# Neptune-Crypto/twenty-first

Hardware: AMD Instinct MI355X
Metric: goldilocks_ntt_gfelts_per_s (higher is better)
Workload: dtype u64

## Files before the change

include/tf_hip.h:

```cpp
#ifndef TF_HIP_H
#define TF_HIP_H

#include <stddef.h>
#include <stdint.h>

#ifdef __cplusplus
extern "C" {
#endif

enum tf_status {
    TF_OK = 0,
    TF_ERR_TOO_FEW_LEAFS = 1,
    TF_ERR_INCORRECT_NUMBER_OF_LEAFS = 2,
    TF_ERR_TREE_TOO_HIGH = 3,
    TF_ERR_LEN_NOT_POWER_OF_TWO = 4,
    TF_ERR_LEN_TOO_LARGE = 5,
    TF_ERR_ORDER_NOT_ABOVE_DEGREE = 6,
    TF_ERR_NULL_POINTER = 7,
    TF_ERR_NO_DEVICE = 8,
    TF_ERR_HIP = 9,
    TF_ERR_OUT_OF_MEMORY = 10,
    TF_ERR_LEAF_INDEX_INVALID = 11,
    TF_ERR_INVERSE_OF_ZERO = 12,
    TF_ERR_BUFFER_TOO_SMALL = 13,
// ... 198 lines not shown
int tf_tip5_sponge_sample_indices(uint64_t *states, size_t count, uint32_t upper_bound, size_t num_indices, uint32_t *out_u32);
int tf_tip5_sponge_sample_indices_dev(uint64_t *d_states, size_t count, uint32_t upper_bound, size_t num_indices, uint32_t *d_out_u32,
                                      void *stream);

int tf_batch_inversion_bfe(const uint64_t *in, size_t n, uint64_t *out);
int tf_batch_inversion_xfe(const uint64_t *in, size_t n, uint64_t *out);
int tf_batch_inversion_bfe_dev(const uint64_t *d_in, size_t n, uint64_t *d_out, void *stream);
int tf_batch_inversion_xfe_dev(const uint64_t *d_in, size_t n, uint64_t *d_out, void *stream);
int tf_batch_inversion_bfe_dev_async(const uint64_t *d_in, size_t n, uint64_t *d_out, void *stream, int *d_status);
int tf_batch_inversion_xfe_dev_async(const uint64_t *d_in, size_t n, uint64_t *d_out, void *stream, int *d_status);
int tf_inverse_or_zero_bfe(const uint64_t *in, size_t n, uint64_t *out);
int tf_inverse_or_zero_xfe(const uint64_t *in, size_t n, uint64_t *out);
int tf_inverse_or_zero_bfe_dev(const uint64_t *d_in, size_t n, uint64_t *d_out, void *stream);
int tf_inverse_or_zero_xfe_dev(const uint64_t *d_in, size_t n, uint64_t *d_out, void *stream);

void tf_set_ntt_tile_bytes(size_t bytes);
size_t tf_get_ntt_tile_bytes(void);
void tf_set_ntt_pipe(int streams);
int tf_get_ntt_pipe(void);

void tf_set_ntt_min_passes(int passes);
void tf_set_ntt_small_launch(int mode);
void tf_set_ntt_two_pass(int mode);
void tf_set_ntt_latency_kernel(int mode);
int tf_ntt_launch_count(size_t n, size_t batch, int width);
int tf_ntt_plan(size_t n, int width, int* log2_radix_out);
double tf_debug_sclk_mhz(void);

#ifdef TF_AB_BUILD
void tf_set_ntt_nt(int mask);
void tf_set_ntt_chain(int tiles_per_workgroup);
int tf_debug_stamps(unsigned long long *host_out, size_t words);
#endif
int tf_debug_fill_random_dev(uint64_t *d_out, size_t count, uint64_t seed, uint64_t first_index, void *stream);

#ifdef __cplusplus
}
#endif
#endif
```

twenty-first_amd/_lib.py:

```python
from __future__ import annotations

import ctypes as C
import os
import subprocess

_HERE = os.path.dirname(os.path.abspath(__file__))
SO_PATH = os.environ.get("TF_HIP_LIBRARY") or os.path.join(_HERE, "libtf_hip.so")
HEADER = os.path.join(os.path.dirname(_HERE), "include", "tf_hip.h")

_u64p = C.POINTER(C.c_uint64)
_sz = C.c_size_t
_vp = C.c_void_p

SIGNATURES = {
    "tf_status_string": (C.c_char_p, [C.c_int]),
    "tf_last_error": (C.c_char_p, []),
    "tf_version": (C.c_int, []),
    "tf_source_hash": (C.c_char_p, []),
    "tf_device_count": (C.c_int, []),
    "tf_set_device": (C.c_int, [C.c_int]),
    "tf_get_device": (C.c_int, [C.POINTER(C.c_int)]),
    "tf_shard_range": (C.c_int, [_sz, C.c_int, C.c_int, C.POINTER(_sz), C.POINTER(_sz)]),
    "tf_merkle_multi_subtrees": (C.c_int, [_sz, _sz, C.c_int]),
    "tf_prepare_ntt": (C.c_int, [_sz, _sz, C.c_int, C.c_int]),
# ... 131 lines not shown
    "tf_tip5_sponge_squeeze": (C.c_int, [_vp, _sz, _sz, _vp]),
    "tf_tip5_sponge_squeeze_dev": (C.c_int, [_vp, _sz, _sz, _vp, _vp]),
    "tf_tip5_sponge_sample_scalars": (C.c_int, [_vp, _sz, _sz, _vp]),
    "tf_tip5_sponge_sample_scalars_dev": (C.c_int, [_vp, _sz, _sz, _vp, _vp]),
    "tf_tip5_sponge_sample_indices": (C.c_int, [_vp, _sz, C.c_uint32, _sz, _vp]),
    "tf_tip5_sponge_sample_indices_dev": (C.c_int, [_vp, _sz, C.c_uint32, _sz, _vp, _vp]),
    "tf_merkle_verify_proofs": (C.c_int, [_vp, _sz, _vp, _vp, _vp, _vp, _vp, _vp, _vp]),
    "tf_merkle_verify_proofs_dev": (C.c_int, [_vp, _sz, _vp, _vp, _vp, _vp, _vp, _vp, _vp, _vp]),
    "tf_merkle_authentication_paths": (C.c_int, [_vp, _sz, _vp, _vp, _vp, _vp, _vp, _vp, _vp]),
    "tf_merkle_authentication_paths_dev": (C.c_int, [_vp, _sz, _vp, _vp, _vp, _vp, _vp, _vp, _vp, _vp]),
    "tf_ntt_launch_count": (C.c_int, [_sz, _sz, C.c_int]),
    "tf_ntt_plan": (C.c_int, [_sz, C.c_int, C.POINTER(C.c_int)]),
    "tf_batch_eval_plan": (C.c_int, [_sz, _sz, _sz, C.c_int]),
    "tf_poly_interpolate_bfe_dev_async": (C.c_int, [_vp, _vp, _sz, _sz, _vp, _vp, _vp]),
    "tf_poly_interpolate_xfe_dev_async": (C.c_int, [_vp, _vp, _sz, _sz, _vp, _vp, _vp]),
    "tf_poly_clean_divide_bfe_dev_async": (C.c_int, [_vp, _sz, _vp, _sz, _vp, _vp, _vp]),
    "tf_poly_clean_divide_many_bfe_dev_async": (C.c_int, [_vp, _sz, _sz, _vp, _sz, _vp, _vp, _vp]),
    "tf_zerofier_tree_new_bfe_dev_async": (C.c_int, [_vp, _sz, _vp, C.POINTER(C.c_void_p)]),
    "tf_zerofier_tree_new_xfe_dev_async": (C.c_int, [_vp, _sz, _vp, C.POINTER(C.c_void_p)]),
    "tf_zerofier_tree_interpolate_dev_async": (C.c_int, [_vp, _vp, _sz, _vp, _vp, _vp]),
    "tf_release_caches": (C.c_int, []),
    "tf_set_ntt_small_launch": (None, [C.c_int]),
    "tf_set_ntt_two_pass": (None, [C.c_int]),
    "tf_set_ntt_latency_kernel": (None, [C.c_int]),
    "tf_debug_sclk_mhz": (C.c_double, []),
    "tf_set_ntt_tile_bytes": (None, [_sz]),
    "tf_set_ntt_min_passes": (None, [C.c_int]),
    "tf_get_ntt_tile_bytes": (_sz, []),
    "tf_set_ntt_pipe": (None, [C.c_int]),
    "tf_get_ntt_pipe": (C.c_int, []),
    "tf_set_batch_eval_route": (None, [C.c_int]),
    "tf_debug_fill_random_dev": (C.c_int, [_vp, _sz, C.c_uint64, C.c_uint64, _vp]),
}


AB_SIGNATURES = {
    "tf_set_ntt_chain": (None, [C.c_int]),
    "tf_debug_stamps": (C.c_int, [_vp, _sz]),
    "tf_set_ntt_nt": (None, [C.c_int]),
}


def build(force: bool = False) -> str:
    csrc = os.path.join(_HERE, "csrc")
    args = ["make", "-C", csrc]
    if force:
# ... 57 lines not shown
```

twenty-first_amd/csrc/ntt_kernels.h:

```cpp
#pragma once

#include <type_traits>

#include "gl64.h"
#include "ntt_args.h"
#include "ntt_network.h"

namespace tfk {

using gl::u32;
using gl::u64;

struct NttPassArgs {
    const u64* in;
    u64* out;
    const u64* inner_tw;
    const u64* post_tw;
    const u64* pre_scale;
    long long n_out;
    const u64* in2;
    const u64* post_scale;
    long long js_i0, js_i1, js_i2, js_c, js_k;
    long long n_coeffs;
    long long ps_i1;
// ... 147 lines not shown
                           Pre2Slot<INV, Q0 + 3>::neg ? v3[3] : v2[3]};
        const u64 m0[4] = {Pre2Slot<INV, Q0>::neg ? v0[0] : v1[0], Pre2Slot<INV, Q0 + 1>::neg ? v0[1] : v1[1], Pre2Slot<INV, Q0 + 2>::neg ? v0[2] : v1[2],
                           Pre2Slot<INV, Q0 + 3>::neg ? v0[3] : v1[3]};
        const u64 m1[4] = {Pre2Slot<INV, Q0>::neg ? v2[0] : v3[0], Pre2Slot<INV, Q0 + 1>::neg ? v2[1] : v3[1], Pre2Slot<INV, Q0 + 2>::neg ? v2[2] : v3[2],
                           Pre2Slot<INV, Q0 + 3>::neg ? v2[3] : v3[3]};
        gl::add_lazy4(p0, p1, t);
        gl::sub_lazy4(t, m0, u);
        gl::sub_lazy4(u, m1, t);
        pre4_shift4<INV, Q0>(x, t);
    } else {
        constexpr int E4 = TwExp<INV, 2, 1>::value;
        gl::sub_lazy4(v0, v2, t);
        gl::sub_lazy4(v1, v3, u);
        const u64 w[4] = {gl::Pow2Mul<E4>::apply(u[0]), gl::Pow2Mul<E4>::apply(u[1]), gl::Pow2Mul<E4>::apply(u[2]), gl::Pow2Mul<E4>::apply(u[3])};
        if ((cls == 1) != gl::Pow2Mul<E4>::negate) gl::add_lazy4(t, w, u);
        else gl::sub_lazy4(t, w, u);
        const u64 b4[4] = {stw[brev5(Q0)], stw[brev5(Q0 + 1)], stw[brev5(Q0 + 2)], stw[brev5(Q0 + 3)]};
        gl::mont_mul4(u, b4, t);
        x[Q0] = t[0], x[Q0 + 1] = t[1], x[Q0 + 2] = t[2], x[Q0 + 3] = t[3];
    }
}
#endif

template <bool INV, int SCALE, int MODE = 0, bool LAST1024 = false, bool R1024 = false, bool COL = false, bool PRE2 = false, bool PRE4 = false>
#ifndef TF_PRIO_LOAD
#define TF_PRIO_LOAD 3
#endif
#ifndef TF_PRIO_STEP2
#define TF_PRIO_STEP2 0
#endif
#ifndef TF_NTT_WAVES
#define TF_NTT_WAVES 4
#endif
__global__ void __launch_bounds__(512, TF_NTT_WAVES) ntt_pass_kernel(const NttPassArgs A) {
    extern __shared__ __attribute__((aligned(16))) u64 lds[];
    const int t = threadIdx.x;
    const int p2 = (LAST1024 || R1024) ? 5 : A.p2;
    const int P2 = 1 << p2;
    constexpr bool COLP = R1024 || COL;
    constexpr bool LAZY1 = (LAST1024 || COLP) && MODE != 2;
    constexpr bool LAZY2 = COLP && MODE == 0;
    const int L = A.L;

    static_assert(!PRE2 || ((LAST1024 || R1024) && MODE == 0 && SCALE != 3), "PRE2 is a variant of the R = 1024 kernels");
    static_assert(!PRE4 || (LAST1024 && !PRE2 && !INV && MODE == 0 && SCALE == 0), "PRE4 is a variant of the plain forward R = 1024 last pass");
#ifndef TF_AB_BUILD
    static_assert(!PRE4, "the radix-4 last pass is a measured loss: laboratory build only");
#endif
    u32 bid = blockIdx.x, half = 0;
    if constexpr (PRE2) {
        if (A.pre2_map == 1) half = (bid >> 3) & 1u, bid = (bid & 7u) | ((bid >> 4) << 3);
        else half = bid & 1u, bid >>= 1;
    }
    if constexpr (PRE4) {
        if (A.pre2_map == 1) half = (bid >> 3) & 3u, bid = (bid & 7u) | ((bid >> 5) << 3);
        else half = bid & 3u, bid >>= 2;
    }
    u32 i0, i1, i2;
    if (A.xcd_order) {
        const u32 G = (u32)A.xcd_order;
        const u32 xcd = bid & 7u, slot = bid >> 3;
        const u32 ngrp = A.d2 / (8u * G);
        const u32 grp = A.xcd_colfast ? slot % ngrp : slot / (G * A.d01);
        const u32 within = A.xcd_colfast ? slot / ngrp : slot % (G * A.d01);
#ifndef TF_XCD_SKEW
#define TF_XCD_SKEW 0
#endif
#ifndef TF_NAT_SKEW
#define TF_NAT_SKEW 0
#endif
        i2 = ((grp << 3) | (TF_XCD_SKEW ? ((xcd + grp * TF_XCD_SKEW) & 7u) : xcd)) * G + within % G;
        const u32 rest = within / G;
        i1 = rest % A.d1;
        i0 = rest / A.d1;
    } else {
        const u32 tile = bid;
        i2 = tile % A.d2;
        const u32 rest = tile / A.d2;
        i1 = rest % A.d1;
        i0 = rest / A.d1;
        if (TF_NAT_SKEW && (A.d2 & 7u) == 0) i2 = (i2 & ~7u) | ((i2 + (i2 >> 3) * TF_NAT_SKEW + rest * TF_NAT_SKEW) & 7u);
    }
    const u64* in = A.in + (long long)i0 * A.ib0 + (long long)i1 * A.ib1 + (long long)i2 * A.ib2;
    u64* out = A.out + (long long)i0 * A.ob0 + (long long)i1 * A.ob1 + (long long)i2 * A.ob2;
    const bool wt = LAST1024 || A.wtiles;
    const int cshift = LAST1024 ? (int)((A.col_shift0 + i0 * (u32)A.col_shift_i0) & 15u) : 0;
    constexpr bool GEO = R1024;
    const int nc_ = GEO ? kR1024Nc : A.nc;
    const int cpr_ = GEO ? kR1024Cpr : A.cpr, nrounds_ = GEO ? kR1024Rounds : A.nrounds;
    const int s1_ = GEO ? kR1024S1 : A.s1, s2_ = GEO ? kR1024Cpr : A.s2, s3_ = GEO ? 1 : A.s3;
    const int col0 = (int)i2 * nc_ - cshift;
    const int ncv = min(nc_, A.col_limit - col0);
    const int ch0 = wt ? (int)div_by_L((u32)max(col0, 0), L) : 0;
    if (wt) {
        in = A.in + (long long)i0 * A.ib0 + (long long)i1 * A.ib1 + (long long)ch0 * A.in_cs_hi;
        out = A.out + (long long)i0 * A.ob0 + (long long)i1 * A.ob1 + (long long)ch0 * A.out_cs_hi;
    }
    if constexpr (PRE2 || PRE4) out += (long long)half * A.pre2_out_off;

    const int g = (LAST1024 || GEO) ? (t >> 4) : (A.gfast ? (t & (P2 - 1)) : (A.nc == 1 ? t : (int)__umulhi((u32)t, A.nc_magic)));
    const int c = (LAST1024 || GEO) ? (t & 15) : (A.gfast ? (t >> p2) : (t - g * A.nc));
    const bool act = c < ncv;
    int ch, cl;
    if (wt) {
        const int w = col0 + c + ((LAST1024 && col0 + c < 0) ? A.col_wrap : 0);
        const int e = (int)div_by_L((u32)w, L);
        ch = e - ch0, cl = w - e * L;
    } else {
        ch = (int)div_by_L((u32)c, L), cl = c - ch * L;
    }
    const long long bcol = (long long)div_by_L((u32)max(col0 + c, 0), L);
    int g_in = LAST1024 ? ((t & 7) | ((t >> 1) & 0x18)) : g;
    int c_in = LAST1024 ? (((t >> 6) & 7) | (t & 8)) : c;
#ifndef TF_XFE_ROLES
#define TF_XFE_ROLES 1
#endif
    if constexpr (LAST1024 && TF_XFE_ROLES) {
        if (L == 3 && col0 >= 0) {
            const int r = (t >> 3) & 1;
            const int v = (t & 7) | ((t >> 4) << 3);
            const int wc0 = col0 + 8 * r;
            int nk = 3 - (wc0 - 3 * (int)div_by_L((u32)wc0, 3));
            int start = 0, colbase = 0;
#pragma unroll
            for (int k = 0; k < 3; ++k) {
                if (v >= start + 32 * nk) {
                    start += 32 * nk;
                    colbase += nk;
                    nk = min(3, 8 - colbase);
                }
            }
            const int local = v - start;
            const int gq = nk == 1 ? local : (nk == 2 ? (local >> 1) : (int)__umulhi((u32)local, 0x55555556u));
            g_in = gq;
            c_in = 8 * r + colbase + (local - gq * nk);
        }
    }
    const bool act_in = LAST1024 ? (c_in < ncv) : act;
    int ch_in = ch, cl_in = cl;
    if constexpr (LAST1024) {
        const int w = col0 + c_in + (col0 + c_in < 0 ? A.col_wrap : 0);
        const int e = (int)div_by_L((u32)w, L);
        ch_in = e - ch0, cl_in = w - e * L;
    }

    unsigned long long stamp[6];
    if constexpr (MODE == 3) stamp[0] = __builtin_readcyclecounter();
    u64 x[32];
#pragma unroll
    for (int q = 0; q < 32; ++q) x[q] = 0;
    constexpr bool LDS_TW = TF_LDS_TW && MODE == 0;
    u64* const ltw = lds + (LAST1024 ? kL1024ExchangeWords : 32 * s1_);
    if constexpr (LDS_TW) {
        if ((LAST1024 || R1024) || A.inner_tw) {
            const u64* itw = A.inner_tw + ((PRE2 || PRE4) ? (int)half * 1024 : 0);
            for (int i = t; i < 32 * P2; i += blockDim.x) ltw[(i >> 5) * kLdsTwStride + (i & 31)] = itw[i];
            __syncthreads();
        }
    }
    __builtin_amdgcn_s_setprio(TF_PRIO_LOAD);
    if constexpr (MODE == 1) {
#pragma unroll
        for (int q = 0; q < 32; ++q) x[q] = (u64)(t * 32 + q) * 0x9e3779b97f4a7c15ULL >> 1;
#ifdef TF_AB_BUILD
    } else if (PRE4 && act_in) {
        const u32 toff = (u32)(((long long)ch_in * A.in_cs_hi + cl_in + (long long)g_in * A.in_rs) * 8);
        const __amdgpu_buffer_rsrc_t ri = buf_rsrc(in);
        const u32 poff = (u32)(A.pre2_in_off * 8);
        const auto slot_off = [&](int q) { return (u32)((long long)(brev5(q) << p2) * A.in_rs * 8); };
        const auto ld = [&](u32 so) { return buf_load<0>(ri, toff, so); };
        const u64* stw = A.pre4_stw + (half >> 1) * 32;
        const auto group = [&](auto q0c) {
            constexpr int Q0 = decltype(q0c)::value;
            u64 v0[4], v1[4], v2[4], v3[4];
#pragma unroll
            for (int i = 0; i < 4; ++i) {
                const u32 so = slot_off(Q0 + i);
                v0[i] = ld(so), v1[i] = ld(so + poff), v2[i] = ld(so + 2 * poff), v3[i] = ld(so + 3 * poff);
            }
            pre4_combine4<INV, Q0>(x, v0, v1, v2, v3, half, stw);
        };
        group(std::integral_constant<int, 0>{});
        group(std::integral_constant<int, 4>{});
// ... 112 lines not shown
        }
        } else {
#pragma unroll
        for (int q = 0; q < 32; ++q) x[q] = ld(slot_off(q));
#pragma unroll
        for (int q0 = 0; q0 < 32; q0 += 8) {
            u64 w[8];
#pragma unroll
            for (int i = 0; i < 8; ++i) w[i] = ld(slot_off(q0 + i) + poff);
            scale8(w);
            if (q0 == 0) pre2_combine8<INV, 0>(x, w, half != 0);
            else if (q0 == 8) pre2_combine8<INV, 8>(x, w, half != 0);
            else if (q0 == 16) pre2_combine8<INV, 16>(x, w, half != 0);
            else pre2_combine8<INV, 24>(x, w, half != 0);
        }
        }
    } else if (act_in) {
        const u32 toff = (u32)(((long long)ch_in * A.in_cs_hi + cl_in + (long long)g_in * A.in_rs) * 8);
        const char* base = reinterpret_cast<const char*>(in);
        if constexpr ((LAST1024 || COLP) && SCALE != 1) {
            const __amdgpu_buffer_rsrc_t ri = buf_rsrc(in);
#pragma unroll
            for (int q = 0; q < 32; ++q) x[q] = buf_load<LAST1024 ? TF_AUX_LAST_LOAD : TF_LOAD_AUX>(ri, toff, (u32)((long long)(brev5(q) << p2) * A.in_rs * 8));
        } else
#pragma unroll
        for (int q = 0; q < 32; ++q) {
            const long long ur = (long long)(brev5(q) << p2);
            const u64* ptr = reinterpret_cast<const u64*>(base + ur * A.in_rs * 8 + toff);
            if constexpr (SCALE == 1) {
                const long long j = (ur + g) * A.ps_rs + (A.ps_col ? bcol : 0);
                if (A.n_coeffs < 0 || j < A.n_coeffs) x[q] = *ptr;
            } else {
#ifdef TF_AB_BUILD
                x[q] = (A.nt & 1) ? __builtin_nontemporal_load(ptr) : *ptr;
#else
                x[q] = *ptr;
#endif
            }
        }
    }
    if constexpr (SCALE == 1) {
        if (act_in && A.in2) {
            const char* base2 = reinterpret_cast<const char*>(in + (A.in2 - A.in));
            const u32 toff2 = (u32)(((long long)ch_in * A.in_cs_hi + cl_in + (long long)g_in * A.in_rs) * 8);
#pragma unroll
            for (int q0 = 0; q0 < 32; q0 += 8) {
// ... 18 lines not shown
                    const long long j = (ur + g) * A.ps_rs + (A.ps_col ? bcol : 0);
                    w[i] = ps[j < A.n_coeffs ? j : 0];
                }
#pragma unroll
                for (int i = 0; i < 8; i += 4) mul4_inplace(x, q0 + i, w[i], w[i + 1], w[i + 2], w[i + 3]);
            }
        }
    }
    if constexpr (PRE2 && !(TF_PRE2_BURST16 == 2 && SCALE != 1)) {
        if (half && act_in) pre2_shift<INV>(x);
    }
    __builtin_amdgcn_s_setprio(0);
    if constexpr (MODE != 2 && !(PRE2 && TF_PRE2_BURST16 == 2 && SCALE != 1)) {
        dit_half<INV, 0, LAZY1>(x);
        __builtin_amdgcn_sched_barrier(0);
    }
    if constexpr (MODE == 3) {
        stamp[1] = __builtin_readcyclecounter();
        asm volatile("s_waitcnt vmcnt(0)" ::: "memory");
        stamp[2] = __builtin_readcyclecounter();
    }
    if constexpr (MODE != 2) {
        dit_half<INV, 16, LAZY1>(x);
        dit_level<INV, 5, LAZY1>(x);
        if ((LAST1024 || R1024) || A.inner_tw) {
            const u64* tw = LDS_TW ? ltw + g_in * kLdsTwStride : A.inner_tw + g_in * 32;
#pragma unroll
            for (int q = 0; q < 32; q += 4) mul4_inplace(x, q, tw[q], tw[q + 1], tw[q + 2], tw[q + 3]);
        }
    }
    if constexpr (MODE == 3) { asm volatile("" :: "v"(x[0]), "v"(x[31])); stamp[3] = __builtin_readcyclecounter(); }
    if constexpr (LAST1024) {
        constexpr int S1 = kL1024S1, CS = kL1024CS;
        const int wround = c_in >> 3, wcc = c_in & 7, rround = c >> 3, rcc = c & 7;
        u64* wr = lds + wcc * CS + g_in;
        const u64* rd = lds + g * S1 + rcc * CS;
        const int nr = (A.nc + 7) >> 3;
#pragma unroll 1
        for (int r = 0; r < nr; ++r) {
            if (r) __syncthreads();
            if (wround == r) {
#pragma unroll
                for (int q = 0; q < 32; ++q) wr[q * S1] = x[q];
            }
            __syncthreads();
            if (rround == r) {
#pragma unroll
                for (int q = 0; q < 32; ++q) x[q] = rd[brev5(q)];
            }
        }
    } else if (p2 != 0) {
        const int myround = c / cpr_;
        const int cc = c - myround * cpr_;
        u64* wr = lds + g * s2_ + cc * s3_;
        const u64* rd = lds + cc * s3_;
#pragma unroll 1
        for (int r = 0; r < nrounds_; ++r) {
            if (r) __syncthreads();
            if (myround == r) {
#pragma unroll
// ... 10 lines not shown
                    x[q] = rd[k1 * s1_ + gg * s2_];
                }
            }
        }
    }
    if constexpr (MODE == 3) { asm volatile("" :: "v"(x[0]), "v"(x[31])); stamp[4] = __builtin_readcyclecounter(); }
    __builtin_amdgcn_s_setprio(TF_PRIO_STEP2);
    if constexpr (LAST1024) {
        dit_half<INV, 0>(x);
        dit_half<INV, 16>(x);
        const u32 toff = (u32)(((long long)ch * A.out_cs_hi + cl + (long long)g * A.out_rs) * 8);
        char* base = reinterpret_cast<char*>(out);
        if constexpr (SCALE == 2) {
            long long j0 = (long long)i0 * A.js_i0 + (long long)i1 * A.js_i1 + (long long)(ch0 + ch) * A.js_c + (long long)g * A.js_k;
            if constexpr (PRE2) j0 += (long long)half * A.pre2_js_off;
            const char* sb = reinterpret_cast<const char*>(A.post_scale);
            const u32 soff = (u32)(j0 * 8);
            tail_p5<INV, 0, false, true>(x, act, base, toff, A.out_rs * 8, 32, sb, soff, A.js_k * 8);
            tail_p5<INV, 4, false, true>(x, act, base, toff, A.out_rs * 8, 32, sb, soff, A.js_k * 8);
            tail_p5<INV, 8, false, true>(x, act, base, toff, A.out_rs * 8, 32, sb, soff, A.js_k * 8);
            tail_p5<INV, 12, false, true>(x, act, base, toff, A.out_rs * 8, 32, sb, soff, A.js_k * 8);
            return;
        }
        if (A.n_out >= 0) {
            const long long j0 = (long long)i0 * A.js_i0 + (long long)i1 * A.js_i1 + (long long)(ch0 + ch) * A.js_c + (long long)g * A.js_k;
            const long long rem = A.n_out - j0, step = 32 * A.js_k;
            const int qlim = rem <= 0 ? 0 : (int)min(32ll, (rem + step - 1) / step);
            tail_p5<INV, 0, true>(x, act, base, toff, A.out_rs * 8, qlim);
            tail_p5<INV, 4, true>(x, act, base, toff, A.out_rs * 8, qlim);
            tail_p5<INV, 8, true>(x, act, base, toff, A.out_rs * 8, qlim);
            tail_p5<INV, 12, true>(x, act, base, toff, A.out_rs * 8, qlim);
            return;
        }
        const bool nts = (A.nt & 2) != 0;
        tail_p5<INV, 0>(x, act, base, toff, A.out_rs * 8, 32, nullptr, 0, 0, nts);
        tail_p5<INV, 4>(x, act, base, toff, A.out_rs * 8, 32, nullptr, 0, 0, nts);
        tail_p5<INV, 8>(x, act, base, toff, A.out_rs * 8, 32, nullptr, 0, 0, nts);
        tail_p5<INV, 12>(x, act, base, toff, A.out_rs * 8, 32, nullptr, 0, 0, nts);
        return;
    }
    if constexpr (MODE != 2) {
        if (p2 >= 1) dit_level<INV, 1, LAZY2>(x);
        if (p2 >= 2) dit_level<INV, 2, LAZY2>(x);
        if (p2 >= 3) dit_level<INV, 3, LAZY2>(x);
        if (p2 >= 4) dit_level<INV, 4, LAZY2>(x);
        if (p2 >= 5) dit_level<INV, 5, LAZY2>(x);
    }
// ... 944 lines not shown
```

twenty-first_amd/csrc/tf_abi.hip:

```cpp
#include "tf_internal.h"
#include "aux_kernels.h"

#include <functional>

namespace tfi {

struct DevBuf {
    u64* p = nullptr;
    hipStream_t s;
    explicit DevBuf(hipStream_t st) : s(st) {}
    int alloc(size_t words) {
        if (words == 0) return TF_OK;
        hipError_t e = pool_malloc_async(reinterpret_cast<void**>(&p), words * sizeof(u64), s);
        if (e != hipSuccess) return hip_fail(e, "hipMallocAsync", __FILE__, __LINE__);
        return TF_OK;
    }
    ~DevBuf() {
        if (p) (void)hipFreeAsync(p, s);
    }
};

int h2d(u64* d, const u64* h, size_t words, hipStream_t s) {
    if (!words) return TF_OK;
    HIPCHK(hipMemcpyAsync(d, h, words * sizeof(u64), hipMemcpyHostToDevice, s));
// ... 227 lines not shown
    return TF_OK;
} TF_ABI_CATCH

#ifdef TF_AB_BUILD
int tf_debug_stamps(unsigned long long* host_out, size_t words) try {
    if (!g_dbg_buf) {
        if (hipMalloc(reinterpret_cast<void**>(&g_dbg_buf), 4096 * 8 * 6 * 8) != hipSuccess) return TF_ERR_HIP;
        (void)hipMemset(g_dbg_buf, 0, 4096 * 8 * 6 * 8);
    }
    if (host_out && words) {
        if (hipDeviceSynchronize() != hipSuccess) return TF_ERR_HIP;
        if (hipMemcpy(host_out, g_dbg_buf, std::min<size_t>(words, 4096 * 8 * 6) * 8, hipMemcpyDeviceToHost) != hipSuccess) return TF_ERR_HIP;
    }
    return TF_OK;
} TF_ABI_CATCH
#endif

void tf_set_ntt_min_passes(int passes) { g_min_passes.store(passes, std::memory_order_relaxed); }
#ifdef TF_AB_BUILD
void tf_set_ntt_chain(int tiles_per_workgroup) { g_chain.store(std::max(0, tiles_per_workgroup), std::memory_order_relaxed); }
#endif
void tf_set_ntt_latency_kernel(int mode) { g_lat_mode.store(mode < 0 ? -1 : (mode ? 1 : 0), std::memory_order_relaxed); }
void tf_set_ntt_two_pass(int mode) { g_pre2_mode.store(mode < 0 ? -1 : (mode > 3 ? 1 : mode), std::memory_order_relaxed); }
void tf_set_ntt_small_launch(int mode) { g_small_launch_mode.store(mode < 0 ? -1 : (mode ? 1 : 0), std::memory_order_relaxed); }
int tf_batch_eval_plan(size_t n_coeffs, size_t n_points, size_t batch, int width) {
    if (width != 1 && width != 3) return 0;
    return tree_route(n_coeffs, n_points, batch, width) ? 2 : 1;
}
int tf_ntt_plan(size_t n, int width, int* log2_radix_out) {
    if (check_len(n) || n <= 1 || (width != 1 && width != 3) || !log2_radix_out) return 0;
    const int log_n = ilog2(n);
    for (int i = 0; i < 4; ++i) log2_radix_out[i] = 0;
    static const bool no_block = ab_env("TF_NTT_NO_BLOCK") != nullptr;
    static const bool no_xfe_block = ab_env("TF_NTT_NO_XFE_BLOCK") != nullptr;
    if (log_n <= 10 || (log_n <= (width == 1 ? 14 : (no_xfe_block ? 10 : 12)) && !no_block && g_min_passes.load(std::memory_order_relaxed) == 0)) {
        log2_radix_out[0] = log_n;
        return 1;
    }
    int P = pass_count(log_n);
    int a[4] = {0, 0, 0, 0};
    choose_split(log_n, P, width, a);
    if (pre2_plan_ok(log_n, width, n, 1, false, -1, false, false, false)) P = 2, pre2_split(log_n, a);
    for (int i = 0; i < P; ++i) log2_radix_out[i] = a[i];
    return P;
}

// ... 766 lines not shown
```

twenty-first_amd/csrc/tf_internal.h:

```cpp
#pragma once
#include <hip/hip_runtime.h>

#include <algorithm>
#include <atomic>
#include <cstdio>
#include <cstdlib>
#include <cstring>
#include <map>
#include <memory>
#include <mutex>
#include <set>
#include <string>
#include <vector>

#pragma GCC visibility push(default)
#include "../../include/tf_hip.h"
#pragma GCC visibility pop
#include "gl64.h"
#include "ntt_args.h"
#include "tf_guard.h"

namespace tfi {

using gl::u32;
// ... 40 lines not shown
    std::vector<ScratchBlock> scratch_free;
    size_t scratch_bytes = 0;
    size_t cached_post_bytes = 0;
    size_t cached_pow_bytes = 0;
    std::map<const u64*, ScratchBlock> temp_pow;
};

constexpr int kMaxDevices = 64;
extern DeviceCtx g_ctx[kMaxDevices];

int current_ctx(DeviceCtx** out);
int device_cus();
hipError_t pool_malloc_async(void** p, size_t bytes, hipStream_t stream);
int scratch_acquire(DeviceCtx* ctx, size_t bytes, hipStream_t stream, DeviceCtx::ScratchBlock* out);
void scratch_release(DeviceCtx* ctx, DeviceCtx::ScratchBlock blk, hipStream_t stream);
int release_caches(DeviceCtx* ctx);
void read_env();
int ensure_dynamic_lds(const void* fn, int bytes, std::atomic<unsigned long long>& done_mask);
int get_pow_table(DeviceCtx* ctx, u64 offset_raw, size_t n, hipStream_t stream, const u64** out, bool* temp, size_t cosets = 1, int log_order = 0);
void release_pow_table(DeviceCtx* ctx, const u64* table, bool temp, hipStream_t stream);

constexpr int kMaxPipe = 4;
extern size_t g_tile_bytes;
extern std::atomic<int> g_pipe, g_nt, g_min_passes, g_lat_mode, g_pre2_mode, g_small_launch_mode;
#ifdef TF_AB_BUILD
extern std::atomic<int> g_chain;
extern unsigned long long* g_dbg_buf;
#endif

enum : u64 { TAG_INNER = 1, TAG_POST = 2, TAG_TINY = 3, TAG_BLOCK1 = 4, TAG_BLOCK2 = 5, TAG_LAT = 6 };
inline u64 make_key(u64 tag, u64 a, u64 b, u64 c, u64 d) { return (tag << 56) | (a << 40) | (b << 24) | (c << 8) | d; }
int upload_table(const std::vector<u64>& host, u64** dev);
int get_post_table(DeviceCtx* ctx, int log_m, int a, bool inverse, hipStream_t stream, const u64** out, bool* temp);

int check_len(size_t n);
int pass_count(int log_n);
void choose_split(int log_n, int P, int L, int (&a)[4]);
void pre2_split(int log_n, int (&a)[4]);
void pre2_split(int log_n, int (&a)[4], bool c8);
bool pre2_plan_ok(int log_n, int L, size_t n, size_t cosets, bool has_in2, long long n_out, bool inverse, bool load_work, bool store_scale);
bool can_truncate(size_t n, int L);
int run_ntt(DeviceCtx* ctx, const u64* in, u64* out, long long in_bs, long long out_bs, size_t n, size_t batch, int L, bool inverse,
            const u64* pre_scale, long long n_coeffs, hipStream_t stream, const u64* post_scale = nullptr, size_t cosets = 1,
            const u64* in2 = nullptr, long long n_out = -1, const u64* coset_offset = nullptr);
int ntt_dev(u64* d_x, size_t n, size_t batch, int L, int inverse, void* stream);
int coset_eval_dev(const u64* d_coeffs, size_t n_coeffs, u64 offset_raw, u64* d_out, size_t order, size_t batch, int L, void* stream);
bool small_launch_for(size_t n, size_t cosets, size_t batch, int L, long long n_out);
// ... 120 lines not shown
```

twenty-first_amd/csrc/tf_ntt.hip:

```cpp
#include "tf_internal.h"
#include "ntt_kernels.h"

namespace tfi {


thread_local std::string t_last_error;

int hip_fail(hipError_t e, const char* what, const char* file, int line) {
    char buf[512];
    snprintf(buf, sizeof(buf), "%s failed: %s (%s:%d)", what, hipGetErrorString(e), file, line);
    t_last_error = buf;
    (void)hipGetLastError();
    if (e == hipErrorNoDevice || e == hipErrorInvalidDevice || e == hipErrorInsufficientDriver || e == hipErrorNotInitialized)
        return TF_ERR_NO_DEVICE;
    if (e == hipErrorOutOfMemory || e == hipErrorMemoryAllocation) return TF_ERR_OUT_OF_MEMORY;
    return TF_ERR_HIP;
}

int abi_caught(const char* what, int status) noexcept {
    try {
        t_last_error = std::string("C++ exception at the C ABI: ") + (what ? what : "?");
    } catch (...) {
    }
    return status;
// ... 870 lines not shown
        A.gfast = 1;
        A.s2 = 1;
        A.s3 = P2;
        A.s1 = pad_to_residue(P2 * A.cpr, 1);
        l.lds_bytes = size_t(32) * A.s1 * sizeof(u64);
    }
    l.tiles = A.d2;
    return l;
}

std::mutex g_func_attr_mutex;
int ensure_dynamic_lds(const void* fn, int bytes, std::atomic<unsigned long long>& done_mask) {
    int dev = 0;
    HIPCHK(hipGetDevice(&dev));
    const unsigned long long bit = 1ull << (dev & 63);
    if (done_mask.load(std::memory_order_acquire) & bit) return TF_OK;
    std::lock_guard<std::mutex> guard(g_func_attr_mutex);
    if (done_mask.load(std::memory_order_acquire) & bit) return TF_OK;
    HIPCHK(hipFuncSetAttribute(fn, hipFuncAttributeMaxDynamicSharedMemorySize, bytes));
    done_mask.fetch_or(bit, std::memory_order_release);
    return TF_OK;
}

template <bool INV, int SCALE, int MODE, bool LAST1024 = false, bool R1024 = false, bool COL = false, bool PRE2 = false, bool PRE4 = false>
int launch_pass_t(const Launch& l, hipStream_t stream) {
    static std::atomic<unsigned long long> done_mask{0};
    if (int rc_attr = ensure_dynamic_lds(reinterpret_cast<const void*>(&tfk::ntt_pass_kernel<INV, SCALE, MODE, LAST1024, R1024, COL, PRE2, PRE4>), (int)(160 * 1024), done_mask)) return rc_attr;
    const size_t lds_bytes = l.lds_bytes + ((TF_LDS_TW && !LAST1024 && MODE == 0 && l.a.inner_tw) ? (size_t(1) << l.a.p2) * tfk::kLdsTwStride * sizeof(u64) : 0);
    hipLaunchKernelGGL((tfk::ntt_pass_kernel<INV, SCALE, MODE, LAST1024, R1024, COL, PRE2, PRE4>), dim3(l.tiles), dim3(l.threads), lds_bytes, stream,
                       l.a);
    HIPCHK(hipGetLastError());
    return TF_OK;
}

template <bool INV, int SCALE>
int launch_col2048_t(const Launch& l, hipStream_t stream) {
    static std::atomic<unsigned long long> done_mask{0};
    if (int rc_attr = ensure_dynamic_lds(reinterpret_cast<const void*>(&tfk::ntt_col2048_kernel<INV, SCALE>), (int)(160 * 1024), done_mask)) return rc_attr;
    const size_t lds_bytes = size_t(32) * tfk::kC8S1 * sizeof(u64);
    hipLaunchKernelGGL((tfk::ntt_col2048_kernel<INV, SCALE>), dim3(l.tiles), dim3(512), lds_bytes, stream, l.a);
    HIPCHK(hipGetLastError());
    return TF_OK;
}

#ifdef TF_AB_BUILD
std::atomic<int> g_chain{-1};
int chain_tiles() {
    int v = g_chain.load(std::memory_order_relaxed);
    if (v < 0) {
        const char* e = ab_env("TF_NTT_PERSIST");
        v = e ? std::max(0, atoi(e)) : 0;
        g_chain.store(v, std::memory_order_relaxed);
    }
    return v;
}
template <bool INV>
int launch_chain_t(const Launch& l, int k, hipStream_t stream) {
    static std::atomic<unsigned long long> done_mask{0};
    if (int rc_attr = ensure_dynamic_lds(reinterpret_cast<const void*>(&tfk::ntt_col1024_chain_kernel<INV>), (int)(160 * 1024), done_mask)) return rc_attr;
    const size_t lds_bytes = l.lds_bytes + size_t(32) * tfk::kLdsTwStride * sizeof(u64);
    unsigned grid = (l.tiles + (unsigned)k - 1) / (unsigned)k;
    grid = (grid + 7u) & ~7u;
    grid = std::min(grid, l.tiles);
    hipLaunchKernelGGL((tfk::ntt_col1024_chain_kernel<INV>), dim3(grid), dim3(512), lds_bytes, stream, l.a, l.tiles, (unsigned)k);
    HIPCHK(hipGetLastError());
    return TF_OK;
}
#else
constexpr int chain_tiles() { return 0; }
#endif

#ifdef TF_AB_BUILD
unsigned long long* g_dbg_buf = nullptr;
#endif
constexpr size_t kLast1024LdsBytes = (size_t(tfk::kL1024ExchangeWords) + (TF_LDS_TW ? 32 * tfk::kLdsTwStride : 0)) * sizeof(u64);

int launch_pass(const Launch& l, bool inverse, hipStream_t stream) {
    if (l.tiles == 0) return TF_OK;
    if (l.bad_geometry) {
        t_last_error = "NTT planner self-check failed (thread-to-column division is not exact for this geometry)";
        return TF_ERR_HIP;
    }
    const int g_ablate = ablate_mode();
    if (l.a.p2 == 5 && !l.a.inner_tw) {
        t_last_error = "internal: R = 1024 pass without its inner twiddle table";
        return TF_ERR_HIP;
    }
    const bool fits = fits_buffer_offsets(l);
    const bool std_geo = l.threads == 512 && l.a.nc == tfk::kR1024Nc && l.a.cpr == tfk::kR1024Cpr && l.a.nrounds == tfk::kR1024Rounds &&
                         l.a.s1 == tfk::kR1024S1 && l.a.s2 == tfk::kR1024Cpr && l.a.s3 == 1 && !l.a.gfast;
    const bool plain_last1024 = l.a.p2 == 5 && !l.a.post_tw && !l.a.gfast && !l.a.pre_scale && l.a.n_coeffs < 0 && !l.a.in2 &&
                                (!l.a.post_scale || (inverse && scaled_last1024_enabled())) && last1024_enabled() && fits;
    if (l.a.p2 == 6) {
        const bool geo = l.threads == 512 && l.a.nc == tfk::kC8Nc && l.a.cpr == tfk::kC8Cpr && l.a.nrounds == tfk::kC8Rounds && l.a.s1 == tfk::kC8S1 &&
                         l.a.s2 == tfk::kC8Cpr && l.a.s3 == 1 && !l.a.gfast && !l.a.wtiles;
        const bool load_work = l.a.pre_scale || l.a.n_coeffs >= 0;
        if (!geo || !fits || g_ablate || !l.a.post_tw || !l.a.inner_tw || l.a.in2 || l.a.n_out >= 0 || l.a.post_scale || l.a.pre2_map ||
            (load_work && inverse) || (l.a.pre_scale && l.a.ps_col)) {
// ... 44 lines not shown
    if (l.a.pre_scale || l.a.n_coeffs >= 0 || l.a.in2) {
        static const bool no_r1024_scale = ab_env("TF_NTT_NO_R1024") != nullptr;
        if (inverse) return launch_pass_t<true, 1, 0>(l, stream);
        if (l.a.p2 == 5 && l.a.post_tw && !no_r1024_scale && fits && std_geo) return launch_pass_t<false, 1, 0, false, true>(l, stream);
        if (l.a.post_tw && fits && !l.a.gfast && col_enabled()) return launch_pass_t<false, 1, 0, false, false, true>(l, stream);
        return launch_pass_t<false, 1, 0>(l, stream);
    }
    if (l.a.post_scale) {
        if (plain_last1024) {
            Launch l2 = l;
            l2.lds_bytes = std::max(l.lds_bytes, kLast1024LdsBytes);
            l2.threads = 512;
            return launch_pass_t<true, 2, 0, true>(l2, stream);
        }
        return launch_pass_t<true, 2, 0>(l, stream);
    }
    const bool last1024 = l.a.p2 == 5 && !l.a.post_tw && last1024_enabled() && !l.a.gfast && fits;
    static const bool no_r1024 = ab_env("TF_NTT_NO_R1024") != nullptr;
    const bool r1024 = l.a.p2 == 5 && l.a.post_tw && g_ablate == 0 && !no_r1024 && fits && std_geo;
    if (last1024) {
        Launch l2 = l;
        l2.lds_bytes = std::max(l.lds_bytes, kLast1024LdsBytes);
        l2.threads = 512;
        return inverse ? launch_pass_t<true, 0, 0, true>(l2, stream) : launch_pass_t<false, 0, 0, true>(l2, stream);
    }
    const bool col = l.a.post_tw && !r1024 && fits && !l.a.gfast && g_ablate == 0 && col_enabled();
#ifdef TF_AB_BUILD
    if (r1024 && chain_tiles() > 1 && l.tiles >= 1024 && !l.a.dbg)
        return inverse ? launch_chain_t<true>(l, chain_tiles(), stream) : launch_chain_t<false>(l, chain_tiles(), stream);
#endif
    if (inverse) return r1024 ? launch_pass_t<true, 0, 0, false, true>(l, stream)
                              : (col ? launch_pass_t<true, 0, 0, false, false, true>(l, stream) : launch_pass_t<true, 0, 0>(l, stream));
    if (r1024) return launch_pass_t<false, 0, 0, false, true>(l, stream);
    if (col) return launch_pass_t<false, 0, 0, false, false, true>(l, stream);
#ifdef TF_AB_BUILD
    if (g_ablate == 1) return launch_pass_t<false, 0, 1>(l, stream);
    if (g_ablate == 2) return launch_pass_t<false, 0, 2>(l, stream);
    if (g_ablate == 3) {
        Launch l2 = l;
        l2.a.dbg = g_dbg_buf;
        return launch_pass_t<false, 0, 3>(l2, stream);
    }
#endif
    return launch_pass_t<false, 0, 0>(l, stream);
}

int check_len(size_t n) {
    if (n != 0 && (n & (n - 1))) return TF_ERR_LEN_NOT_POWER_OF_TWO;
    if (n > (size_t(1) << 31)) return TF_ERR_LEN_TOO_LARGE;
    return TF_OK;
}

#ifdef TF_AB_BUILD
// ... 558 lines not shown
```

Baseline: 146.3.

## Add fixed-shape specialization of radix-1024 NTT pass kernels

Adds a FIXED template variant of the plain and last radix-1024 pass kernels that is used when the geometry is power-of-two, unskewed and has full 16-column tiles. In that variant the tile-index decode uses shifts and masks instead of divisions, bounds checks, wrap handling and zero-init are dropped, and the column loop is fixed at two rounds. It also moves the inner twiddle table's LDS fill so the global loads issue alongside the data loads and the LDS stores land between butterfly levels, instead of a separate prologue with its own barrier. This adds more kernel instantiations and a runtime eligibility check, and it relies on the gating predicate being exact.

```diff
diff --git a/include/tf_hip.h b/include/tf_hip.h
--- a/include/tf_hip.h
+++ b/include/tf_hip.h
@@ -244,6 +244,7 @@
 void tf_set_ntt_min_passes(int passes);
 void tf_set_ntt_small_launch(int mode);
 void tf_set_ntt_two_pass(int mode);
+void tf_set_ntt_fixed_shape(int mode);
 void tf_set_ntt_latency_kernel(int mode);
 int tf_ntt_launch_count(size_t n, size_t batch, int width);
 int tf_ntt_plan(size_t n, int width, int* log2_radix_out);
diff --git a/twenty-first_amd/_lib.py b/twenty-first_amd/_lib.py
--- a/twenty-first_amd/_lib.py
+++ b/twenty-first_amd/_lib.py
@@ -177,6 +177,7 @@
     "tf_release_caches": (C.c_int, []),
     "tf_set_ntt_small_launch": (None, [C.c_int]),
     "tf_set_ntt_two_pass": (None, [C.c_int]),
+    "tf_set_ntt_fixed_shape": (None, [C.c_int]),
     "tf_set_ntt_latency_kernel": (None, [C.c_int]),
     "tf_debug_sclk_mhz": (C.c_double, []),
     "tf_set_ntt_tile_bytes": (None, [_sz]),
diff --git a/twenty-first_amd/csrc/ntt_kernels.h b/twenty-first_amd/csrc/ntt_kernels.h
--- a/twenty-first_amd/csrc/ntt_kernels.h
+++ b/twenty-first_amd/csrc/ntt_kernels.h
@@ -193,7 +193,8 @@
 }
 #endif
 
-template <bool INV, int SCALE, int MODE = 0, bool LAST1024 = false, bool R1024 = false, bool COL = false, bool PRE2 = false, bool PRE4 = false>
+template <bool INV, int SCALE, int MODE = 0, bool LAST1024 = false, bool R1024 = false, bool COL = false, bool PRE2 = false, bool PRE4 = false,
+          bool FIXED = false>
 #ifndef TF_PRIO_LOAD
 #define TF_PRIO_LOAD 3
 #endif
@@ -211,7 +212,7 @@
     constexpr bool COLP = R1024 || COL;
     constexpr bool LAZY1 = (LAST1024 || COLP) && MODE != 2;
     constexpr bool LAZY2 = COLP && MODE == 0;
-    const int L = A.L;
+    const int L = FIXED ? 1 : A.L;
 
     static_assert(!PRE2 || ((LAST1024 || R1024) && MODE == 0 && SCALE != 3), "PRE2 is a variant of the R = 1024 kernels");
     static_assert(!PRE4 || (LAST1024 && !PRE2 && !INV && MODE == 0 && SCALE == 0), "PRE4 is a variant of the plain forward R = 1024 last pass");
@@ -227,8 +228,24 @@
         if (A.pre2_map == 1) half = (bid >> 3) & 3u, bid = (bid & 7u) | ((bid >> 5) << 3);
         else half = bid & 3u, bid >>= 2;
     }
+    static_assert(!FIXED || ((LAST1024 != R1024) && SCALE == 0 && MODE == 0 && !COL && !PRE2 && !PRE4), "FIXED is a variant of the two plain R = 1024 kernels");
     u32 i0, i1, i2;
-    if (A.xcd_order) {
+    if constexpr (FIXED) {
+        const u32 d1_sh = (u32)__builtin_ctz(A.d1);
+        u32 rest;
+        if (A.xcd_order) {
+            const u32 xcd = bid & 7u, slot = bid >> 3;
+            const u32 sh = (u32)__builtin_ctz(A.xcd_colfast ? A.d2 >> 3 : A.d01);
+            const u32 lo = slot & ((1u << sh) - 1u), hi = slot >> sh;
+            i2 = ((A.xcd_colfast ? lo : hi) << 3) | xcd;
+            rest = A.xcd_colfast ? hi : lo;
+        } else {
+            i2 = bid & (A.d2 - 1u);
+            rest = bid >> (u32)__builtin_ctz(A.d2);
+        }
+        i1 = rest & (A.d1 - 1u);
+        i0 = rest >> d1_sh;
+    } else if (A.xcd_order) {
         const u32 G = (u32)A.xcd_order;
         const u32 xcd = bid & 7u, slot = bid >> 3;
         const u32 ngrp = A.d2 / (8u * G);
@@ -252,16 +269,17 @@
         i0 = rest / A.d1;
         if (TF_NAT_SKEW && (A.d2 & 7u) == 0) i2 = (i2 & ~7u) | ((i2 + (i2 >> 3) * TF_NAT_SKEW + rest * TF_NAT_SKEW) & 7u);
     }
+    static_assert(!FIXED || (TF_XCD_SKEW == 0 && TF_NAT_SKEW == 0), "the FIXED decode has no skewed tile orders");
     const u64* in = A.in + (long long)i0 * A.ib0 + (long long)i1 * A.ib1 + (long long)i2 * A.ib2;
     u64* out = A.out + (long long)i0 * A.ob0 + (long long)i1 * A.ob1 + (long long)i2 * A.ob2;
-    const bool wt = LAST1024 || A.wtiles;
-    const int cshift = LAST1024 ? (int)((A.col_shift0 + i0 * (u32)A.col_shift_i0) & 15u) : 0;
+    const bool wt = LAST1024 || (!FIXED && A.wtiles);
+    const int cshift = (LAST1024 && !FIXED) ? (int)((A.col_shift0 + i0 * (u32)A.col_shift_i0) & 15u) : 0;
     constexpr bool GEO = R1024;
     const int nc_ = GEO ? kR1024Nc : A.nc;
     const int cpr_ = GEO ? kR1024Cpr : A.cpr, nrounds_ = GEO ? kR1024Rounds : A.nrounds;
     const int s1_ = GEO ? kR1024S1 : A.s1, s2_ = GEO ? kR1024Cpr : A.s2, s3_ = GEO ? 1 : A.s3;
     const int col0 = (int)i2 * nc_ - cshift;
-    const int ncv = min(nc_, A.col_limit - col0);
+    const int ncv = FIXED ? 16 : min(nc_, A.col_limit - col0);
     const int ch0 = wt ? (int)div_by_L((u32)max(col0, 0), L) : 0;
     if (wt) {
         in = A.in + (long long)i0 * A.ib0 + (long long)i1 * A.ib1 + (long long)ch0 * A.in_cs_hi;
@@ -271,10 +289,10 @@
 
     const int g = (LAST1024 || GEO) ? (t >> 4) : (A.gfast ? (t & (P2 - 1)) : (A.nc == 1 ? t : (int)__umulhi((u32)t, A.nc_magic)));
     const int c = (LAST1024 || GEO) ? (t & 15) : (A.gfast ? (t >> p2) : (t - g * A.nc));
-    const bool act = c < ncv;
+    const bool act = FIXED || c < ncv;
     int ch, cl;
     if (wt) {
-        const int w = col0 + c + ((LAST1024 && col0 + c < 0) ? A.col_wrap : 0);
+        const int w = col0 + c + ((LAST1024 && !FIXED && col0 + c < 0) ? A.col_wrap : 0);
         const int e = (int)div_by_L((u32)w, L);
         ch = e - ch0, cl = w - e * L;
     } else {
@@ -307,10 +325,10 @@
             c_in = 8 * r + colbase + (local - gq * nk);
         }
     }
-    const bool act_in = LAST1024 ? (c_in < ncv) : act;
+    const bool act_in = FIXED || (LAST1024 ? (c_in < ncv) : act);
     int ch_in = ch, cl_in = cl;
     if constexpr (LAST1024) {
-        const int w = col0 + c_in + (col0 + c_in < 0 ? A.col_wrap : 0);
+        const int w = col0 + c_in + ((!FIXED && col0 + c_in < 0) ? A.col_wrap : 0);
         const int e = (int)div_by_L((u32)w, L);
         ch_in = e - ch0, cl_in = w - e * L;
     }
@@ -318,11 +336,14 @@
     unsigned long long stamp[6];
     if constexpr (MODE == 3) stamp[0] = __builtin_readcyclecounter();
     u64 x[32];
-#pragma unroll
-    for (int q = 0; q < 32; ++q) x[q] = 0;
+    if constexpr (!FIXED) {
+#pragma unroll
+        for (int q = 0; q < 32; ++q) x[q] = 0;
+    }
     constexpr bool LDS_TW = TF_LDS_TW && MODE == 0;
+    static_assert(!FIXED || LDS_TW, "the FIXED kernels read their inner table from LDS");
     u64* const ltw = lds + (LAST1024 ? kL1024ExchangeWords : 32 * s1_);
-    if constexpr (LDS_TW) {
+    if constexpr (LDS_TW && !FIXED) {
         if ((LAST1024 || R1024) || A.inner_tw) {
             const u64* itw = A.inner_tw + ((PRE2 || PRE4) ? (int)half * 1024 : 0);
             for (int i = t; i < 32 * P2; i += blockDim.x) ltw[(i >> 5) * kLdsTwStride + (i & 31)] = itw[i];
@@ -330,6 +351,7 @@
         }
     }
     __builtin_amdgcn_s_setprio(TF_PRIO_LOAD);
+    u64 tws[2];
     if constexpr (MODE == 1) {
 #pragma unroll
         for (int q = 0; q < 32; ++q) x[q] = (u64)(t * 32 + q) * 0x9e3779b97f4a7c15ULL >> 1;
@@ -488,6 +510,7 @@
             const __amdgpu_buffer_rsrc_t ri = buf_rsrc(in);
 #pragma unroll
             for (int q = 0; q < 32; ++q) x[q] = buf_load<LAST1024 ? TF_AUX_LAST_LOAD : TF_LOAD_AUX>(ri, toff, (u32)((long long)(brev5(q) << p2) * A.in_rs * 8));
+            if constexpr (FIXED) tws[0] = A.inner_tw[t], tws[1] = A.inner_tw[t + 512];
         } else
 #pragma unroll
         for (int q = 0; q < 32; ++q) {
@@ -552,7 +575,12 @@
     }
     if constexpr (MODE != 2) {
         dit_half<INV, 16, LAZY1>(x);
+        if constexpr (FIXED) {
+            ltw[(t >> 5) * kLdsTwStride + (t & 31)] = tws[0];
+            ltw[((t + 512) >> 5) * kLdsTwStride + (t & 31)] = tws[1];
+        }
         dit_level<INV, 5, LAZY1>(x);
+        if constexpr (FIXED) __syncthreads();
         if ((LAST1024 || R1024) || A.inner_tw) {
             const u64* tw = LDS_TW ? ltw + g_in * kLdsTwStride : A.inner_tw + g_in * 32;
 #pragma unroll
@@ -565,7 +593,7 @@
         const int wround = c_in >> 3, wcc = c_in & 7, rround = c >> 3, rcc = c & 7;
         u64* wr = lds + wcc * CS + g_in;
         const u64* rd = lds + g * S1 + rcc * CS;
-        const int nr = (A.nc + 7) >> 3;
+        const int nr = FIXED ? 2 : (A.nc + 7) >> 3;
 #pragma unroll 1
         for (int r = 0; r < nr; ++r) {
             if (r) __syncthreads();
@@ -622,7 +650,7 @@
             tail_p5<INV, 12, false, true>(x, act, base, toff, A.out_rs * 8, 32, sb, soff, A.js_k * 8);
             return;
         }
-        if (A.n_out >= 0) {
+        if (!FIXED && A.n_out >= 0) {
             const long long j0 = (long long)i0 * A.js_i0 + (long long)i1 * A.js_i1 + (long long)(ch0 + ch) * A.js_c + (long long)g * A.js_k;
             const long long rem = A.n_out - j0, step = 32 * A.js_k;
             const int qlim = rem <= 0 ? 0 : (int)min(32ll, (rem + step - 1) / step);
diff --git a/twenty-first_amd/csrc/tf_abi.hip b/twenty-first_amd/csrc/tf_abi.hip
--- a/twenty-first_amd/csrc/tf_abi.hip
+++ b/twenty-first_amd/csrc/tf_abi.hip
@@ -273,6 +273,7 @@
 #endif
 void tf_set_ntt_latency_kernel(int mode) { g_lat_mode.store(mode < 0 ? -1 : (mode ? 1 : 0), std::memory_order_relaxed); }
 void tf_set_ntt_two_pass(int mode) { g_pre2_mode.store(mode < 0 ? -1 : (mode > 3 ? 1 : mode), std::memory_order_relaxed); }
+void tf_set_ntt_fixed_shape(int mode) { g_fixed_mode.store(mode < 0 ? -1 : (mode ? 1 : 0), std::memory_order_relaxed); }
 void tf_set_ntt_small_launch(int mode) { g_small_launch_mode.store(mode < 0 ? -1 : (mode ? 1 : 0), std::memory_order_relaxed); }
 int tf_batch_eval_plan(size_t n_coeffs, size_t n_points, size_t batch, int width) {
     if (width != 1 && width != 3) return 0;
diff --git a/twenty-first_amd/csrc/tf_internal.h b/twenty-first_amd/csrc/tf_internal.h
--- a/twenty-first_amd/csrc/tf_internal.h
+++ b/twenty-first_amd/csrc/tf_internal.h
@@ -86,7 +86,7 @@
 
 constexpr int kMaxPipe = 4;
 extern size_t g_tile_bytes;
-extern std::atomic<int> g_pipe, g_nt, g_min_passes, g_lat_mode, g_pre2_mode, g_small_launch_mode;
+extern std::atomic<int> g_pipe, g_nt, g_min_passes, g_lat_mode, g_pre2_mode, g_small_launch_mode, g_fixed_mode;
 #ifdef TF_AB_BUILD
 extern std::atomic<int> g_chain;
 extern unsigned long long* g_dbg_buf;
diff --git a/twenty-first_amd/csrc/tf_ntt.hip b/twenty-first_amd/csrc/tf_ntt.hip
--- a/twenty-first_amd/csrc/tf_ntt.hip
+++ b/twenty-first_amd/csrc/tf_ntt.hip
@@ -916,12 +916,13 @@
     return TF_OK;
 }
 
-template <bool INV, int SCALE, int MODE, bool LAST1024 = false, bool R1024 = false, bool COL = false, bool PRE2 = false, bool PRE4 = false>
+template <bool INV, int SCALE, int MODE, bool LAST1024 = false, bool R1024 = false, bool COL = false, bool PRE2 = false, bool PRE4 = false,
+          bool FIXED = false>
 int launch_pass_t(const Launch& l, hipStream_t stream) {
     static std::atomic<unsigned long long> done_mask{0};
-    if (int rc_attr = ensure_dynamic_lds(reinterpret_cast<const void*>(&tfk::ntt_pass_kernel<INV, SCALE, MODE, LAST1024, R1024, COL, PRE2, PRE4>), (int)(160 * 1024), done_mask)) return rc_attr;
+    if (int rc_attr = ensure_dynamic_lds(reinterpret_cast<const void*>(&tfk::ntt_pass_kernel<INV, SCALE, MODE, LAST1024, R1024, COL, PRE2, PRE4, FIXED>), (int)(160 * 1024), done_mask)) return rc_attr;
     const size_t lds_bytes = l.lds_bytes + ((TF_LDS_TW && !LAST1024 && MODE == 0 && l.a.inner_tw) ? (size_t(1) << l.a.p2) * tfk::kLdsTwStride * sizeof(u64) : 0);
-    hipLaunchKernelGGL((tfk::ntt_pass_kernel<INV, SCALE, MODE, LAST1024, R1024, COL, PRE2, PRE4>), dim3(l.tiles), dim3(l.threads), lds_bytes, stream,
+    hipLaunchKernelGGL((tfk::ntt_pass_kernel<INV, SCALE, MODE, LAST1024, R1024, COL, PRE2, PRE4, FIXED>), dim3(l.tiles), dim3(l.threads), lds_bytes, stream,
                        l.a);
     HIPCHK(hipGetLastError());
     return TF_OK;
@@ -968,6 +969,20 @@
 unsigned long long* g_dbg_buf = nullptr;
 #endif
 constexpr size_t kLast1024LdsBytes = (size_t(tfk::kL1024ExchangeWords) + (TF_LDS_TW ? 32 * tfk::kLdsTwStride : 0)) * sizeof(u64);
+
+std::atomic<int> g_fixed_mode{-1};
+bool fixed_shape_ok(const Launch& l) {
+    const tfk::NttPassArgs& a = l.a;
+    const auto pow2 = [](u32 v) { return v != 0 && (v & (v - 1)) == 0; };
+    if (g_fixed_mode.load(std::memory_order_relaxed) == 0) return false;
+    if (a.L != 1 || a.p2 != 5 || a.nc != 16 || l.threads != 512 || a.wtiles || a.gfast || a.pre2_map) return false;
+    if (a.col_shift0 || a.col_shift_i0 || a.n_out >= 0 || a.n_coeffs >= 0 || a.pre_scale || a.in2 || a.post_scale || a.dbg) return false;
+    if (a.col_limit <= 0 || (a.col_limit & 15) || (unsigned)a.col_limit != a.d2 * 16u) return false;
+    if (!pow2(a.d1) || !pow2(a.d2)) return false;
+    if (a.xcd_order > 1 || (a.xcd_order == 1 && (a.d2 & 7u))) return false;
+    if (a.xcd_order == 1 && !a.xcd_colfast && !pow2(a.d01)) return false;
+    return true;
+}
 
 int launch_pass(const Launch& l, bool inverse, hipStream_t stream) {
     if (l.tiles == 0) return TF_OK;
@@ -1058,6 +1073,9 @@
         Launch l2 = l;
         l2.lds_bytes = std::max(l.lds_bytes, kLast1024LdsBytes);
         l2.threads = 512;
+        if (fixed_shape_ok(l))
+            return inverse ? launch_pass_t<true, 0, 0, true, false, false, false, false, true>(l2, stream)
+                           : launch_pass_t<false, 0, 0, true, false, false, false, false, true>(l2, stream);
         return inverse ? launch_pass_t<true, 0, 0, true>(l2, stream) : launch_pass_t<false, 0, 0, true>(l2, stream);
     }
     const bool col = l.a.post_tw && !r1024 && fits && !l.a.gfast && g_ablate == 0 && col_enabled();
@@ -1065,6 +1083,9 @@
     if (r1024 && chain_tiles() > 1 && l.tiles >= 1024 && !l.a.dbg)
         return inverse ? launch_chain_t<true>(l, chain_tiles(), stream) : launch_chain_t<false>(l, chain_tiles(), stream);
 #endif
+    if (r1024 && fixed_shape_ok(l))
+        return inverse ? launch_pass_t<true, 0, 0, false, true, false, false, false, true>(l, stream)
+                       : launch_pass_t<false, 0, 0, false, true, false, false, false, true>(l, stream);
     if (inverse) return r1024 ? launch_pass_t<true, 0, 0, false, true>(l, stream)
                               : (col ? launch_pass_t<true, 0, 0, false, false, true>(l, stream) : launch_pass_t<true, 0, 0>(l, stream));
     if (r1024) return launch_pass_t<false, 0, 0, false, true>(l, stream);
```

After: 147.5, median of 6. No clear change (+0.8%).
